# OEmiliatanO/Unpaired-Multimodal-Learning

Measured on NVIDIA B200. Metric: UML train samples/sec (img+text), higher is better.
Workload: dtype bf16

## Files before the change

### unpaired-multimodal-learning_b200/csrc/common.cuh

```cuda
#pragma once

#include <cuda.h>
#include <cuda_bf16.h>
#include <cuda_runtime.h>
#include <stdint.h>

#include <cstdio>
#include <cstring>

#include "../../include/uml_b200.h"

#if defined(__CUDA_ARCH__) && !(defined(__CUDA_ARCH_FEAT_SM100_ALL) || defined(__CUDA_ARCH_SPECIFIC__) || (__CUDA_ARCH__ >= 1000))
#error "libuml_b200 is written for sm_100a only"
#endif

namespace uml {

void set_error(const char* fmt, ...);

#define UML_FAIL(...)            \
  do {                           \
    ::uml::set_error(__VA_ARGS__); \
    return 1;                    \
  } while (0)
// ... 218 lines not shown

__device__ __forceinline__ uint32_t cluster_ctarank() {
  uint32_t r;
  asm volatile("mov.u32 %0, %%cluster_ctarank;" : "=r"(r));
  return r;
}
__device__ __forceinline__ uint32_t mapa_cta(uint32_t saddr, uint32_t rank) {
  uint32_t r;
  asm volatile("mapa.shared::cluster.u32 %0, %1, %2;" : "=r"(r) : "r"(saddr), "r"(rank));
  return r;
}
__device__ __forceinline__ void cluster_sync_all() {
  asm volatile("barrier.cluster.arrive.release.aligned;\n\tbarrier.cluster.wait.acquire.aligned;" ::: "memory");
}
__device__ __forceinline__ void mbar_arrive_remote(uint32_t cluster_addr) {
  asm volatile("mbarrier.arrive.shared::cluster.b64 _, [%0];" ::"r"(cluster_addr) : "memory");
}
__device__ __forceinline__ void tma_load_2d_cg2(void* smem_dst, const CUtensorMap* m, uint32_t bar_cluster_addr,
                                                int32_t c0, int32_t c1) {
  asm volatile(
      "cp.async.bulk.tensor.2d.cta_group::2.shared::cluster.global.mbarrier::complete_tx::bytes [%0], [%1, {%3, %4}], [%2];"
      ::"r"(smem_u32(smem_dst)), "l"(reinterpret_cast<uint64_t>(m)), "r"(bar_cluster_addr), "r"(c0), "r"(c1)
      : "memory");
}
__device__ __forceinline__ void umma_bf16_cg2(uint32_t tmem_d, uint64_t desc_a, uint64_t desc_b, uint32_t idesc,
                                              uint32_t accumulate) {
  asm volatile(
      "{\n\t.reg .pred p;\n\t"
      "setp.ne.b32 p, %4, 0;\n\t"
      "tcgen05.mma.cta_group::2.kind::f16 [%0], %1, %2, %3, p;\n\t}\n" ::"r"(tmem_d),
      "l"(desc_a), "l"(desc_b), "r"(idesc), "r"(accumulate)
      : "memory");
}
__device__ __forceinline__ void umma_commit_cg2(uint64_t* bar) {
  asm volatile(
      "tcgen05.commit.cta_group::2.mbarrier::arrive::one.shared::cluster.multicast::cluster.b64 [%0], %1;" ::"r"(
          smem_u32(bar)),
      "h"(static_cast<uint16_t>(3))
      : "memory");
}
__device__ __forceinline__ void tmem_alloc_cg2(uint32_t* smem_slot, uint32_t cols) {
  asm volatile("tcgen05.alloc.cta_group::2.sync.aligned.shared::cta.b32 [%0], %1;" ::"r"(smem_u32(smem_slot)), "r"(cols)
               : "memory");
  asm volatile("tcgen05.relinquish_alloc_permit.cta_group::2.sync.aligned;" ::: "memory");
}
__device__ __forceinline__ void tmem_dealloc_cg2(uint32_t addr, uint32_t cols) {
  asm volatile("tcgen05.dealloc.cta_group::2.sync.aligned.b32 %0, %1;" ::"r"(addr), "r"(cols) : "memory");
}

__device__ __forceinline__ float warp_sum(float v) {
#pragma unroll
  for (int o = 16; o > 0; o >>= 1) v += __shfl_xor_sync(0xffffffffu, v, o);
  return v;
}
__device__ __forceinline__ float warp_max(float v) {
#pragma unroll
  for (int o = 16; o > 0; o >>= 1) v = fmaxf(v, __shfl_xor_sync(0xffffffffu, v, o));
  return v;
}
__device__ __forceinline__ int warp_sum_i(int v) {
#pragma unroll
  for (int o = 16; o > 0; o >>= 1) v += __shfl_xor_sync(0xffffffffu, v, o);
  return v;
}

#endif

}
```

### unpaired-multimodal-learning_b200/csrc/tc_fwd2.cu

```cuda
#include <cstdlib>
#include <type_traits>

#include "common.cuh"

namespace uml {

#ifndef UML_X_TMAST
#define UML_X_TMAST 1
#endif
constexpr bool kXTmaStore = UML_X_TMAST != 0;
#ifndef UML_X_STAGES
#define UML_X_STAGES (UML_X_TMAST ? 5 : 6)
#endif
constexpr int kXStages = UML_X_STAGES;
constexpr int kXABytes = 128 * 64 * 2;
constexpr int kXBBytes = 128 * 64 * 2;
constexpr int kXStageBytes = kXABytes + kXBBytes;
constexpr int kXRecBytes = 32;
#ifndef UML_X_SLICES
#define UML_X_SLICES 2
#endif
constexpr int kXSlices = UML_X_SLICES;
constexpr int kXSliceCols = 256 / kXSlices;
#ifndef UML_X_GC
#define UML_X_GC 32
#endif
constexpr int kXGC = UML_X_GC;
#ifndef UML_X_DB
#define UML_X_DB 0
#endif
constexpr bool kXDoubleBuf = UML_X_DB != 0;
constexpr int kXGW = kXGC / 2;
constexpr int kXGroups = kXSliceCols / kXGC;
constexpr int kXHxSlots = 4;
constexpr int kXHxBytes = kXHxSlots * (kXSlices - 1) * 128 * kXRecBytes;
constexpr int kXEpiWarpsC = 4 * kXSlices;
constexpr int kXSbufWarp = 2 * 2048;
constexpr int kXSbufBytes = kXTmaStore ? kXEpiWarpsC * kXSbufWarp : 0;
constexpr int kXSmemBytes = kXStages * kXStageBytes + kXSbufBytes + kXHxBytes + 1024  + 256 ;
constexpr int kXEpiWarps = 4 * kXSlices;
constexpr int kXWarpMma = kXEpiWarps, kXWarpTma = kXEpiWarps + 1;
constexpr int kXThreads = (kXEpiWarps + 4) * 32;
#ifndef UML_X_REGS_P
#define UML_X_REGS_P (kXSlices == 2 ? 40 : 24)
#define UML_X_REGS_E (kXSlices == 2 ? 232 : 112)
#endif
constexpr int kXRegsProducer = UML_X_REGS_P, kXRegsEpilogue = UML_X_REGS_E;
static_assert((kXThreads - 128) * (kXRegsEpilogue - 168) <= 128 * (168 - kXRegsProducer) || kXSlices != 2, "setmaxnreg: the epilogue asks for more than the producers free");
#ifndef UML_X_HALF
#define UML_X_HALF (kXGroups > 2 ? kXGroups - 1 : kXGroups / 2)
#endif
constexpr int kXHalf = UML_X_HALF;
constexpr int kXMaxChunks = 4;
#ifndef UML_X_REQ_AFTER
#define UML_X_REQ_AFTER 0
#endif
constexpr int kXReqAfter = UML_X_REQ_AFTER;
static_assert(kXHalf >= 1 && kXHalf <= kXGroups && kXReqAfter < kXHalf, "the records must be requested before they are resolved");
static_assert(kXSmemBytes <= 227 * 1024, "exchange forward kernel: shared memory");

struct XSegs {
  int64_t n0;
  const float* scale_dev[2];
  float scale[2], dcoef[2];
};

struct XWork {
  float* tile_part;
  uint4* recs;
  unsigned* ctrl;
};

__device__ __forceinline__ float x_exp2(float x) {
  float y;
  asm("ex2.approx.ftz.f32 %0, %1;" : "=f"(y) : "f"(x));
  return y;
}
__device__ __forceinline__ void st_volatile_v4(uint4* p, uint32_t a, uint32_t b, uint32_t c, uint32_t d) {
  asm volatile("st.volatile.global.v4.u32 [%0], {%1, %2, %3, %4};" ::"l"(p), "r"(a), "r"(b), "r"(c), "r"(d) : "memory");
}
__device__ __forceinline__ uint4 ld_volatile_v4(const uint4* p) {
  uint4 v;
  asm volatile("ld.volatile.global.v4.u32 {%0, %1, %2, %3}, [%4];" : "=r"(v.x), "=r"(v.y), "=r"(v.z), "=r"(v.w) : "l"(p) : "memory");
  return v;
}
__device__ __forceinline__ void sts128(uint32_t a, uint32_t x, uint32_t y, uint32_t z, uint32_t w) {
  asm volatile("st.shared.v4.b32 [%0], {%1, %2, %3, %4};" ::"r"(a), "r"(x), "r"(y), "r"(z), "r"(w) : "memory");
}
__device__ __forceinline__ void sts64(uint32_t a, uint32_t x, uint32_t y) {
  asm volatile("st.shared.v2.b32 [%0], {%1, %2};" ::"r"(a), "r"(x), "r"(y) : "memory");
}
__device__ __forceinline__ uint4 lds128(uint32_t a) {
  uint4 v;
  asm volatile("ld.shared.v4.b32 {%0, %1, %2, %3}, [%4];" : "=r"(v.x), "=r"(v.y), "=r"(v.z), "=r"(v.w) : "r"(a) : "memory");
  return v;
}
__device__ __forceinline__ uint2 lds64(uint32_t a) {
  uint2 v;
  asm volatile("ld.shared.v2.b32 {%0, %1}, [%2];" : "=r"(v.x), "=r"(v.y) : "r"(a) : "memory");
  return v;
}
__device__ __forceinline__ void stg256(void* p, const uint32_t* w) {
  asm volatile("st.global.v8.b32 [%0], {%1, %2, %3, %4, %5, %6, %7, %8};" ::"l"(p), "r"(w[0]), "r"(w[1]), "r"(w[2]), "r"(w[3]),
               "r"(w[4]), "r"(w[5]), "r"(w[6]), "r"(w[7])
               : "memory");
}
__device__ __forceinline__ void named_bar_sync(int id, int n) { asm volatile("bar.sync %0, %1;" ::"r"(id), "r"(n) : "memory"); }
__device__ __forceinline__ void tmem_ld16(uint32_t taddr, uint32_t (&v)[16]) {
  asm volatile(
      "tcgen05.ld.sync.aligned.32x32b.x16.b32 "
      "{%0, %1, %2, %3, %4, %5, %6, %7, %8, %9, %10, %11, %12, %13, %14, %15}, [%16];"
      : "=r"(v[0]), "=r"(v[1]), "=r"(v[2]), "=r"(v[3]), "=r"(v[4]), "=r"(v[5]), "=r"(v[6]), "=r"(v[7]),
        "=r"(v[8]), "=r"(v[9]), "=r"(v[10]), "=r"(v[11]), "=r"(v[12]), "=r"(v[13]), "=r"(v[14]), "=r"(v[15])
      : "r"(taddr)
      : "memory");
}
__device__ __forceinline__ void tmem_ldg(uint32_t taddr, uint32_t (&v)[16]) { tmem_ld16(taddr, v); }
// ... 43 lines not shown
  case i:           \
    asm volatile("mov.b32 %0, %1;" : "=r"(r) : "r"(v[(i) < N ? (i) : 0])); \
    break;
  switch (d) {
    UML_PICK(0) UML_PICK(1) UML_PICK(2) UML_PICK(3) UML_PICK(4) UML_PICK(5) UML_PICK(6) UML_PICK(7)
    UML_PICK(8) UML_PICK(9) UML_PICK(10) UML_PICK(11) UML_PICK(12) UML_PICK(13) UML_PICK(14) UML_PICK(15)
    UML_PICK(16) UML_PICK(17) UML_PICK(18) UML_PICK(19) UML_PICK(20) UML_PICK(21) UML_PICK(22) UML_PICK(23)
    UML_PICK(24) UML_PICK(25) UML_PICK(26) UML_PICK(27) UML_PICK(28) UML_PICK(29) UML_PICK(30) UML_PICK(31)
    default: break;
  }
#undef UML_PICK
  return __uint_as_float(r);
}

template <int B, int E, class F>
__device__ __forceinline__ void static_for(F&& f) {
  if constexpr (B < E) {
    f(std::integral_constant<int, B>());
    static_for<B + 1, E>(f);
  }
}

template <bool kPred, bool kDs>
__global__ void __launch_bounds__(kXThreads, 1)
    head_fwd_ce_x_kernel(const __grid_constant__ CUtensorMap tmap_x, const __grid_constant__ CUtensorMap tmap_w,
                         const __grid_constant__ CUtensorMap tmap_g,
                         int64_t n_rows, int dim, int n_classes, int n_groups, const int32_t* __restrict__ labels, XSegs segs,
                         uint16_t* __restrict__ G, int64_t ldg, float* __restrict__ row_loss, int32_t* __restrict__ row_pred,
                         int32_t* __restrict__ row_correct, float* __restrict__ row_dscale, XWork wk) {
  extern __shared__ unsigned char smem_raw[];
  unsigned char* smem = reinterpret_cast<unsigned char*>((reinterpret_cast<uintptr_t>(smem_raw) + 1023) & ~uintptr_t(1023));
  unsigned char* sbuf = smem + kXStages * kXStageBytes;
  unsigned char* hx = sbuf + kXSbufBytes;
  uint64_t* full_bar = reinterpret_cast<uint64_t*>(hx + kXHxBytes);
  uint64_t* empty_bar = full_bar + kXStages;
  uint64_t* tfull_bar = empty_bar + kXStages;
  uint64_t* tempty_bar = tfull_bar + 2;
  uint64_t* xbar = tempty_bar + 2;
  uint32_t* tmem_slot = reinterpret_cast<uint32_t*>(xbar + 4);
  uint32_t* epoch_slot = tmem_slot + 1;
  float* run_scale = reinterpret_cast<float*>(epoch_slot + 1);

  const int warp = threadIdx.x >> 5, lane = threadIdx.x & 31;
  const uint32_t rank = cluster_ctarank();
  const bool leader = rank == 0;
  const int num_kb = (dim + 63) / 64;
  const int n_chunks = (n_classes + 255) / 256;
  const int pair = blockIdx.x >> 1;
  const int chunk = pair % n_chunks, group = pair / n_chunks;
  const int col0 = chunk * 256;
  const int n_valid = n_classes - col0 < 256 ? n_classes - col0 : 256;
  const int n_mma = ((n_valid + 15) / 16) * 16;
  const int64_t n_units = (n_rows + 255) / 256;
  const bool write_g = G != nullptr;

  if (warp == kXWarpTma && lane == 0) {
    tma_prefetch_desc(&tmap_x);
    tma_prefetch_desc(&tmap_w);
    if (kXTmaStore && write_g) tma_prefetch_desc(&tmap_g);
  }
  if (warp == kXWarpMma && lane == 0) {
    for (int s = 0; s < kXStages; ++s) {
      mbar_init(&full_bar[s], 2);
      mbar_init(&empty_bar[s], 1);
    }
    for (int b = 0; b < 2; ++b) {
      mbar_init(&tfull_bar[b], 1);
      mbar_init(&tempty_bar[b], 2 * kXEpiWarps);
    }
    for (int qq = 0; qq < 4; ++qq) mbar_init(&xbar[qq], kXSlices - 1);
    fence_barrier_init();
  }
  if (warp == kXWarpTma) tmem_alloc_cg2(tmem_slot, 512);
  tc_fence_before();
  cluster_sync_all();
  tc_fence_after();
  const uint32_t tmem_base = *tmem_slot;
  pdl_trigger();
  pdl_wait();
  if (threadIdx.x < 2) run_scale[threadIdx.x] = segs.scale_dev[threadIdx.x] ? __ldg(segs.scale_dev[threadIdx.x]) : segs.scale[threadIdx.x];
  if (threadIdx.x == 0) {
    *epoch_slot = *reinterpret_cast<volatile unsigned*>(wk.ctrl) + 1u;
    if (blockIdx.x == 0) wk.ctrl[3] = gridDim.x * 4u;
  }
  __syncthreads();
  const unsigned epoch = *epoch_slot;

  if (warp >= kXEpiWarps) {
    asm volatile("setmaxnreg.dec.sync.aligned.u32 %0;" ::"n"(kXRegsProducer));
  if (warp == kXWarpTma) {
    if (lane == 0) {
      uint32_t it = 0;
      XDBG_DECL();
      const uint32_t lead_bar0 = mapa_cta(smem_u32(&full_bar[0]), 0);
      const int32_t wrow0 = col0 + static_cast<int32_t>(rank) * (n_mma / 2);
      for (int64_t unit = group; unit < n_units; unit += n_groups) {
        const int32_t row0 = static_cast<int32_t>((unit * 2 + rank) * 128);
        for (int kb = 0; kb < num_kb; ++kb, ++it) {
          const uint32_t s = it % kXStages, ph = (it / kXStages) & 1;
          XDBG_MARK();
          mbar_wait(&empty_bar[s], ph ^ 1);
          XDBG_ACC(0);
          unsigned char* a = smem + s * kXStageBytes;
          const uint32_t lead_bar = lead_bar0 + s * 8;
#ifdef UML_X_HALFLOAD
          if (leader) mbar_arrive_expect_tx(&full_bar[s], 2 * kXBBytes);
#else
          if (leader) mbar_arrive_expect_tx(&full_bar[s], 2 * kXStageBytes);
          tma_load_2d_cg2(a, &tmap_x, lead_bar, kb * 64, row0);
#endif
          tma_load_2d_cg2(a + kXABytes, &tmap_w, lead_bar, kb * 64, wrow0);
          if (!leader) mbar_arrive_remote(lead_bar);
          XDBG_ACC(1);
        }
      }
      XDBG_FLUSH(12, 2);
    }
    __syncwarp();
  } else if (warp == kXWarpMma) {
    if (lane == 0 && leader) {
      const uint32_t idesc = make_idesc_bf16(256, static_cast<uint32_t>(n_mma), 0, 0);
      uint32_t it = 0, acc_it = 0;
      XDBG_DECL();
      for (int64_t unit = group; unit < n_units; unit += n_groups, ++acc_it) {
        const uint32_t b = acc_it & 1, aph = (acc_it >> 1) & 1;
        XDBG_MARK();
        mbar_wait(&tempty_bar[b], aph ^ 1);
        XDBG_ACC(0);
        tc_fence_after();
        const uint32_t d_tmem = tmem_base + b * 256;
        for (int kb = 0; kb < num_kb; ++kb, ++it) {
          const uint32_t s = it % kXStages, ph = (it / kXStages) & 1;
          mbar_wait(&full_bar[s], ph);
          XDBG_ACC(1);
          tc_fence_after();
          const uint32_t a_addr = smem_u32(smem + s * kXStageBytes);
          const uint32_t b_addr = a_addr + kXABytes;
#pragma unroll
          for (int k = 0; k < 4; ++k) {
            const uint64_t da = make_smem_desc(a_addr + k * 32, 16, 1024, kLayoutSw128);
            const uint64_t db = make_smem_desc(b_addr + k * 32, 16, 1024, kLayoutSw128);
            umma_bf16_cg2(d_tmem, da, db, idesc, (kb | k) != 0);
          }
          umma_commit_cg2(&empty_bar[s]);
          XDBG_ACC(2);
        }
        umma_commit_cg2(&tfull_bar[b]);
      }
      XDBG_FLUSH(9, 3);
    }
    __syncwarp();
  }
  } else {
    asm volatile("setmaxnreg.inc.sync.aligned.u32 %0;" ::"n"(kXRegsEpilogue));
    const int q = warp & 3;
    const int cq = warp >> 2;
    constexpr float kLog2e = 1.4426950408889634f;
    constexpr float kMasked = -1.0e30f;
    constexpr bool kSecond = kPred || kDs;
    const int rloc = q * 32 + lane;
    const uint32_t hx_base = smem_u32(hx);
    const uint32_t tempty_remote0 = mapa_cta(smem_u32(&tempty_bar[0]), 0);
    const int live_groups = !write_g ? 0 : static_cast<int>((ldg - col0 - cq * kXSliceCols) / kXGC);
    uint32_t tile_it = 0;
    XDBG_DECL();

    struct RowCtx {
      float sl2, sabs, sgn, dcoef, gcoef;
      bool valid, sg;
    };
    const float scale_a = run_scale[0], scale_b = run_scale[1];
    const bool any_neg = scale_a < 0.f || scale_b < 0.f;
    auto row_ctx = [&](int64_t row) {
      RowCtx c;
      c.valid = row < n_rows;
      c.sg = c.valid && row >= segs.n0;
      const float scale = c.sg ? run_scale[1] : run_scale[0];
      c.dcoef = c.sg ? segs.dcoef[1] : segs.dcoef[0];
      c.gcoef = c.dcoef * scale;
      c.sgn = scale < 0.f ? -1.f : 1.f;
      c.sabs = fabsf(scale);
      c.sl2 = c.sabs * kLog2e;
      return c;
    };

    uint32_t pk[kXSliceCols / 2];
    float p_gm[kXGroups];
#pragma unroll
    for (int g = 0; g < kXGroups; ++g) p_gm[g] = 0.f;
    float p_before = 0.f, p_lraw = 0.f, p_lab_p = 0.f, p_lab_gm = 0.f;
    int p_label = -1;
    int p_tile = -1;
    const uint4* p_rec = wk.recs;
    float f_M = 0.f, f_tc = 0.f, f_sl2 = 0.f;
    unsigned short f_patch = 0;
    bool f_store = false;
    unsigned char* f_grow = nullptr;
    float acc_loss[2] = {0.f, 0.f}, acc_ds[2] = {0.f, 0.f};
    int acc_hit[2] = {0, 0}, acc_cnt[2] = {0, 0};

    uint4 r0[kXMaxChunks], r1[kXMaxChunks];
    auto request_prev = [&]() {
      if (static_cast<int64_t>(p_tile) * 128 + rloc < n_rows) {
#pragma unroll
        for (int c2 = 0; c2 < kXMaxChunks; ++c2) {
          if (c2 < n_chunks) {
            r0[c2] = ld_volatile_v4(p_rec + c2 * 2);
            if (kSecond) r1[c2] = ld_volatile_v4(p_rec + c2 * 2 + 1);
          }
        }
      }
    };
    auto resolve_prev = [&]() {
      const int64_t row = static_cast<int64_t>(p_tile) * 128 + rloc;
      const RowCtx c = row_ctx(row);
      float M = -INFINITY, S = 0.f, PR = 0.f, before_chunks = -INFINITY;
      int garg = 0x7fffffff;
      if (c.valid) {
        for (unsigned polls = 0;; ++polls) {
          bool fresh = true;
#pragma unroll
          for (int c2 = 0; c2 < kXMaxChunks; ++c2) {
            if (c2 < n_chunks) {
              fresh = fresh && r0[c2].y == epoch && r0[c2].w == epoch;
              if (kSecond) fresh = fresh && r1[c2].y == epoch && r1[c2].w == epoch;
            }
          }
          if (fresh) break;
          if (polls > (1u << 20)) {
            atomicExch(wk.ctrl + 2, 1u);
            break;
          }
          request_prev();
        }
        float om[kXMaxChunks], os[kXMaxChunks];
#pragma unroll
        for (int c2 = 0; c2 < kXMaxChunks; ++c2) {
          om[c2] = c2 < n_chunks ? __uint_as_float(r0[c2].x) : -INFINITY;
          os[c2] = c2 < n_chunks ? __uint_as_float(r0[c2].z) : 0.f;
          M = fmaxf(M, om[c2]);
          if (c2 < chunk) before_chunks = fmaxf(before_chunks, om[c2]);
        }
        const float offM = __fmul_rn(M, c.sl2);
#pragma unroll
        for (int c2 = 0; c2 < kXMaxChunks; ++c2) {
          const float e = x_exp2(__fmul_rn(om[c2], c.sl2) - offM);
          S = fmaf(os[c2], e, S);
          if (kDs) PR = fmaf(c2 < n_chunks ? __uint_as_float(r1[c2].x) : 0.f, e, PR);
        }
        if (kPred) {
          float bestm = -INFINITY;
#pragma unroll
          for (int c2 = 0; c2 < kXMaxChunks; ++c2) {
            if (c2 < n_chunks && om[c2] > bestm) {
              bestm = om[c2];
              garg = static_cast<int>(r1[c2].z);
            }
          }
        }
      }
      f_M = __fmul_rn(M, c.sl2);
      f_sl2 = c.sl2;
      f_tc = __fdividef(c.gcoef, S);
      f_store = c.valid && live_groups > 0;
      f_grow = reinterpret_cast<unsigned char*>(G) + (row * ldg + col0 + cq * kXSliceCols) * 2;
      {
        const float f = x_exp2(__fmul_rn(p_lab_gm, c.sl2) - f_M) * f_tc;
        f_patch = __bfloat16_as_ushort(__float2bfloat16_rn(fmaf(p_lab_p, f, -c.gcoef)));
      }
      if (cq == 0) {
        const int lc_chunk = p_label - col0;
        if (c.valid && lc_chunk >= 0 && lc_chunk < 256) {
          const float loss = fmaxf(fmaf(__log2f(S), 0.6931471805599453f, -0.6931471805599453f * fmaf(p_lraw, c.sl2, -f_M)), 0.f);
          const float dsc = kDs ? (__fdividef(PR, S) - p_lraw) * c.sgn * c.dcoef : 0.f;
          const int hit = (p_lraw == M && p_lraw > fmaxf(before_chunks, p_before)) ? 1 : 0;
          if (row_loss) row_loss[row] = loss;
          if (kPred && row_pred) row_pred[row] = garg;
          if (row_correct) row_correct[row] = hit;
          if (kDs && row_dscale) row_dscale[row] = dsc;
          if (c.sg) { acc_loss[1] += loss; acc_ds[1] += dsc; acc_hit[1] += hit; acc_cnt[1] += 1; }
          else { acc_loss[0] += loss; acc_ds[0] += dsc; acc_hit[0] += hit; acc_cnt[0] += 1; }
        }
      }
    };
    auto finish_group = [&](auto gc) {
      constexpr int g = decltype(gc)::value;
      if (!f_store || g >= live_groups) return;
      const float gmx = p_gm[g];
      const float f = x_exp2(__fmul_rn(gmx, f_sl2) - f_M) * f_tc;
// ... 32 lines not shown
      }
      const uint32_t box = sbuf_w + (g & 1) * 2048, rowb = box + lane * 64, sw = (lane >> 1) & 3;
      if (lane == 0) bulk_wait_read<1>();
      __syncwarp();
#pragma unroll
      for (int j4 = 0; j4 < kXGW / 4; ++j4) sts128(rowb + ((j4 ^ sw) << 4), o[4 * j4], o[4 * j4 + 1], o[4 * j4 + 2], o[4 * j4 + 3]);
      const int lc = p_label - col0 - cq * kXSliceCols - g * kXGC;
      if (static_cast<unsigned>(lc) < static_cast<unsigned>(kXGC))
        asm volatile("st.shared.u16 [%0], %1;" ::"r"(rowb + (((lc >> 3) ^ sw) << 4) + (lc & 7) * 2), "h"(f_patch) : "memory");
      fence_proxy_async();
      __syncwarp();
#ifndef UML_X_NOSTORE
      if (lane == 0) {
        asm volatile("cp.async.bulk.tensor.2d.global.shared::cta.bulk_group [%0, {%2, %3}], [%1];" ::"l"(
                         reinterpret_cast<uint64_t>(&tmap_g)),
                     "r"(box), "r"(col0 + cq * kXSliceCols + g * kXGC), "r"(p_tile * 128 + q * 32)
                     : "memory");
        bulk_commit();
      }
#endif
    };
    auto finish_any = [&](auto gc) {
      if constexpr (kXTmaStore) finish_group_tma(gc);
      else finish_group(gc);
    };
    auto finish_rows = [&]() {
      if (kXTmaStore) return;
      const int lcol = p_label - col0 - cq * kXSliceCols;
      if (f_store && lcol >= 0 && lcol < kXSliceCols) *reinterpret_cast<volatile unsigned short*>(f_grow + lcol * 2) = f_patch;
    };

    int next_label = -1;
    {
      const int64_t frow = (static_cast<int64_t>(group) * 2 + rank) * 128 + rloc;
      if (group < n_units && frow < n_rows) next_label = __ldg(labels + frow);
    }
    for (int unit = group; unit < static_cast<int>(n_units); unit += n_groups, ++tile_it) {
      const int tile = unit * 2 + static_cast<int>(rank);
      const int64_t row = static_cast<int64_t>(tile) * 128 + rloc;
      const RowCtx c = row_ctx(row);
      const float sl2 = c.sl2, sgn = c.sgn;
      const int label = next_label;
      {
        const int64_t nrow = (static_cast<int64_t>(unit + n_groups) * 2 + rank) * 128 + rloc;
        next_label = nrow < n_rows ? __ldg(labels + nrow) : -1;
      }
#ifdef UML_X_NOLABEL
      const int lcol = -1000000;
#else
      const int lcol = label - col0 - cq * kXSliceCols;
#endif
      float run_max = -INFINITY, run_sum = 0.f, run_pr = 0.f, max_before = -INFINITY, lab_raw = -INFINITY;
      float lab_p = 0.f, lab_gm = 0.f;
      int arg = 0x7fffffff;
      float gm[kXGroups];
      const bool have_prev = p_tile >= 0;

      const uint32_t b = tile_it & 1, aph = (tile_it >> 1) & 1;
      XDBG_MARK();
      mbar_wait(&tfull_bar[b], aph);
      XDBG_ACC(0);
      tc_fence_after();
#ifdef UML_X_NOEPI
      tc_fence_before();
      __syncwarp();
      if (lane == 0) {
        if (!leader) mbar_arrive_remote(tempty_remote0 + b * 8);
        else mbar_arrive(&tempty_bar[b]);
      }
      continue;
#endif
      const uint32_t taddr = tmem_base + (static_cast<uint32_t>(q * 32) << 16) + b * 256 + cq * kXSliceCols;
      uint32_t vv[kXDoubleBuf ? 2 : 1][kXGC];
      uint32_t nk[kXGW * kXHalf];

      const uint64_t sl2x2 = pack2(sl2, sl2);
      auto run_group = [&](uint32_t (&v)[kXGC], uint32_t* out, auto gc) -> float {
// ... 69 lines not shown
          out[j] = *reinterpret_cast<const uint32_t*>(&hh);
        }
        float s0, s1;
        unpack2(fadd2(sx2, sy2), s0, s1);
        run_sum += s0 + s1;
        if (kDs) run_pr += q0 + q1;
        if (lab_here) {
          lab_p = __bfloat162float(__float2bfloat16_rn(x_exp2(__fmaf_rn(lab_raw, sl2, noff))));
          lab_gm = new_max;
        }
        return new_max;
      };

      constexpr int kB = kXDoubleBuf ? 1 : 0;
      tmem_ldg(taddr, vv[0]);
      static_for<0, kXGroups>([&](auto gc) {
        constexpr int g = decltype(gc)::value;
        constexpr bool last = g == kXGroups - 1;
        tmem_ld_wait();
        pin16(vv[g & kB]);
        if (g == 0) XDBG_ACC(1);
        if (last) {
          tc_fence_before();
          __syncwarp();
          if (lane == 0) {
            if (!leader) mbar_arrive_remote(tempty_remote0 + b * 8);
            else mbar_arrive(&tempty_bar[b]);
          }
        } else if (kXDoubleBuf) {
          tmem_ldg(taddr + kXGC * (g + 1), vv[(g + 1) & kB]);
        }
        gm[g] = run_group(vv[g & kB], g < kXHalf ? nk + kXGW * g : pk + kXGW * g, gc);
        if (!last && !kXDoubleBuf) tmem_ldg(taddr + kXGC * (g + 1), vv[0]);
        if (g == kXReqAfter && have_prev) request_prev();
        if (g == kXHalf - 1) {
          if (have_prev) {
            resolve_prev();
            static_for<0, (kXHalf + 1 < kXGroups ? kXHalf + 1 : kXGroups)>([&](auto fc) { finish_any(fc); });
          }
#pragma unroll
          for (int j = 0; j < kXGW * kXHalf; ++j) pk[j] = nk[j];
        } else if (g >= kXHalf && !last) {
          if (have_prev) finish_any(std::integral_constant<int, g + 1>());
        }
      });
      XDBG_ACC(2);
      if (have_prev) finish_rows();
      XDBG_ACC(3);

      const uint32_t hx_slot = hx_base + (tile_it & (kXHxSlots - 1)) * ((kXSlices - 1) * 128 * kXRecBytes);
      const uint4* rec_row = wk.recs + row * n_chunks * 2;
      if (cq != 0) {
        const uint32_t mine = hx_slot + ((cq - 1) * 128 + rloc) * kXRecBytes;
        sts128(mine, __float_as_uint(run_max), __float_as_uint(run_sum), __float_as_uint(max_before), __float_as_uint(lab_raw));
        if (kSecond) sts64(mine + 16, __float_as_uint(run_pr), static_cast<uint32_t>(arg));
        __syncwarp();
        if (lane == 0) mbar_arrive(&xbar[q]);
      } else {
        mbar_wait(&xbar[q], tile_it & 1);
        float cm = run_max, before_loc = max_before, lraw = lab_raw;
        constexpr int kOthers = kXSlices - 1;
        float o_max[kOthers], o_sum[kOthers], o_pr[kOthers];
        int o_arg[kOthers];
#pragma unroll
        for (int k = 0; k < kOthers; ++k) {
          const uint32_t other = hx_slot + (k * 128 + rloc) * kXRecBytes;
          const uint4 o4 = lds128(other);
          o_max[k] = __uint_as_float(o4.x);
          o_sum[k] = __uint_as_float(o4.y);
          cm = fmaxf(cm, o_max[k]);
          before_loc = fmaxf(before_loc, __uint_as_float(o4.z));
          lraw = fmaxf(lraw, __uint_as_float(o4.w));
          o_pr[k] = 0.f;
          o_arg[k] = 0;
          if (kSecond) {
            const uint2 o2 = lds64(other + 16);
            o_pr[k] = __uint_as_float(o2.x);
            o_arg[k] = static_cast<int>(o2.y);
          }
        }
        const float offc = __fmul_rn(cm, sl2);
        const float e_me = x_exp2(__fmul_rn(run_max, sl2) - offc);
        float cs = run_sum * e_me, cpr = kDs ? run_pr * e_me : 0.f;
#pragma unroll
        for (int k = 0; k < kOthers; ++k) {
          const float e = x_exp2(__fmul_rn(o_max[k], sl2) - offc);
          cs = fmaf(o_sum[k], e, cs);
          if (kDs) cpr = fmaf(o_pr[k], e, cpr);
        }
        int carg = arg;
        if (kPred) {
          float bmx = run_max;
#pragma unroll
          for (int k = 0; k < kOthers; ++k) {
            if (o_max[k] > bmx) {
              bmx = o_max[k];
              carg = o_arg[k];
            }
          }
        }
        if (c.valid) {
          uint4* rec = const_cast<uint4*>(rec_row) + chunk * 2;
          st_volatile_v4(rec, __float_as_uint(cm), epoch, __float_as_uint(cs), epoch);
          if (kSecond) st_volatile_v4(rec + 1, __float_as_uint(cpr), epoch, static_cast<uint32_t>(carg), epoch);
        }
        p_before = before_loc;
        p_lraw = lraw;
      }
      XDBG_ACC(4);
#pragma unroll
      for (int g = 0; g < kXGroups; ++g) p_gm[g] = gm[g];
      p_lab_p = lab_p; p_lab_gm = lab_gm;
      p_label = label; p_tile = tile; p_rec = rec_row;
    }
    if (p_tile >= 0) {
      XDBG_MARK();
      request_prev();
      resolve_prev();
      XDBG_ACC(5);
      static_for<0, kXGroups>([&](auto gc) { finish_any(gc); });
      finish_rows();
      XDBG_ACC(6);
    }
    if (kXTmaStore && lane == 0) bulk_wait<0>();
    if (cq == 0 && wk.tile_part) {
#pragma unroll
      for (int s2 = 0; s2 < 2; ++s2) {
        const float a = warp_sum(acc_loss[s2]), dd = kDs ? warp_sum(acc_ds[s2]) : 0.f;
        const int hh = warp_sum_i(acc_hit[s2]), cnt = warp_sum_i(acc_cnt[s2]);
        if (lane == 0)
          *reinterpret_cast<float4*>(wk.tile_part + ((static_cast<int64_t>(blockIdx.x) * 4 + q) * 2 + s2) * 4) =
              make_float4(a, dd, static_cast<float>(hh), static_cast<float>(cnt));
      }
    }
#ifdef UML_FWD_TIMING
    if (warp == 0 && lane == 0) XDBG_FLUSH(0, 9);
#endif
  }

  tc_fence_before();
  cluster_sync_all();
  if (warp == kXWarpTma) tmem_dealloc_cg2(tmem_base, 512);
  if (threadIdx.x == 0) {
    __threadfence();
    const unsigned done = atomicAdd(wk.ctrl + 1, 1u);
    if (done == gridDim.x - 1) {
      wk.ctrl[1] = 0u;
      __threadfence();
      *reinterpret_cast<volatile unsigned*>(wk.ctrl) = epoch;
    }
  }
}

__global__ void __launch_bounds__(1024)
    x_tile_stats_kernel(const float* __restrict__ tile_part, int64_t n_entries, uml_seg_stats* __restrict__ out) {
  pdl_trigger();
  pdl_wait();
  __shared__ float sh[4][32];
  const int s = blockIdx.x;
  float acc[4] = {0.f, 0.f, 0.f, 0.f};
  for (int64_t i = threadIdx.x; i < n_entries; i += blockDim.x) {
    const float* p = tile_part + (i * 2 + s) * 4;
#pragma unroll
    for (int k = 0; k < 4; ++k) acc[k] += p[k];
  }
#pragma unroll
  for (int k = 0; k < 4; ++k) {
    const float v = warp_sum(acc[k]);
    if ((threadIdx.x & 31) == 0) sh[k][threadIdx.x >> 5] = v;
  }
  __syncthreads();
  if (threadIdx.x == 0) {
    float tot[4] = {0.f, 0.f, 0.f, 0.f};
    for (int k = 0; k < 4; ++k)
      for (int w = 0; w < static_cast<int>(blockDim.x >> 5); ++w) tot[k] += sh[k][w];
    out[s].loss_mean = tot[3] > 0.f ? tot[0] / tot[3] : 0.f;
    out[s].dscale = tot[1];
    out[s].correct = static_cast<int32_t>(tot[2] + 0.5f);
    out[s].n = static_cast<int32_t>(tot[3] + 0.5f);
  }
}

__global__ void __launch_bounds__(1024)
    x_tile_stats_dev_kernel(const float* __restrict__ tile_part, const unsigned* __restrict__ ctrl, uml_seg_stats* __restrict__ out) {
  pdl_trigger();
  pdl_wait();
  __shared__ float sh[4][32];
  const int s = blockIdx.x;
  const int64_t n_entries = ctrl[3];
  float acc[4] = {0.f, 0.f, 0.f, 0.f};
  for (int64_t i = threadIdx.x; i < n_entries; i += blockDim.x) {
    const float* p = tile_part + (i * 2 + s) * 4;
#pragma unroll
    for (int k = 0; k < 4; ++k) acc[k] += p[k];
  }
#pragma unroll
  for (int k = 0; k < 4; ++k) {
    const float v = warp_sum(acc[k]);
    if ((threadIdx.x & 31) == 0) sh[k][threadIdx.x >> 5] = v;
  }
  __syncthreads();
  if (threadIdx.x == 0) {
    float tot[4] = {0.f, 0.f, 0.f, 0.f};
    for (int k = 0; k < 4; ++k)
      for (int w = 0; w < static_cast<int>(blockDim.x >> 5); ++w) tot[k] += sh[k][w];
    out[s].loss_mean = tot[3] > 0.f ? tot[0] / tot[3] : 0.f;
    out[s].dscale = tot[1];
    out[s].correct = static_cast<int32_t>(tot[2] + 0.5f);
    out[s].n = static_cast<int32_t>(tot[3] + 0.5f);
  }
}

struct XLayout {
  unsigned* ctrl;
  float* tile_part;
  uint4* recs;
  int64_t part_entries;
  int64_t n_groups;
};
static XLayout x_layout(float* tile_ws, int64_t n_rows, int n_classes) {
  const int64_t units = (n_rows + 255) / 256;
  const int n_chunks = (n_classes + 255) / 256;
  XLayout l;
  l.ctrl = reinterpret_cast<unsigned*>(tile_ws);
  l.tile_part = tile_ws + 16 + units * 8;
  l.recs = reinterpret_cast<uint4*>(l.tile_part + units * 256);
  l.n_groups = (sm_count() / 2) / n_chunks;
  if (l.n_groups > units) l.n_groups = units;
  l.part_entries = l.n_groups * n_chunks * 2 * 4;
  return l;
}

}

bool uml_fwd_x_eligible(int64_t n_rows, int32_t n_classes) {
  static int mode = -1;
  if (mode < 0) {
    const char* e = getenv("UML_FWD_IMPL");
    mode = (e && e[0] == 'o') ? 0 : 1;
  }
  return mode == 1 && n_rows > 128 && n_classes <= uml::kXMaxChunks * 256;
}

void uml_fwd_x_partials(float* tile_ws, int64_t n_rows, int32_t n_classes, const float** part, int64_t* n_entries) {
  const uml::XLayout l = uml::x_layout(tile_ws, n_rows, n_classes);
  *part = l.tile_part;
  *n_entries = l.part_entries;
}

int uml_head_fwd_ce_x_bf16(const uint16_t* X, int64_t n_rows, int32_t dim, const uint16_t* W, int32_t n_classes,
                           const int32_t* labels, const uml_tc_segments* segs, uint16_t* G, int64_t ldg, float* row_loss,
                           int32_t* row_pred, int32_t* row_correct, float* row_dscale, float* tile_ws, uml_seg_stats* stats,
                           void* stream) {
  using namespace uml;
  UML_REQUIRE(X && W && labels && segs && tile_ws && n_rows > 0 && dim > 0 && n_classes > 0, "head_fwd_ce_x: bad arguments");
  UML_REQUIRE(dim % 8 == 0, "head_fwd_ce_x: dim (%d) must be a multiple of 8 (16-byte bf16 rows for TMA)", dim);
  UML_REQUIRE(n_classes <= kXMaxChunks * 256, "head_fwd_ce_x: at most %d classes", kXMaxChunks * 256);
  UML_REQUIRE(!G || (ldg % 64 == 0 && ldg >= n_classes && ldg <= kXMaxChunks * 256),
              "head_fwd_ce_x: ldg must be a multiple of 64 and >= n_classes");
  UML_REQUIRE(segs->nseg >= 1 && segs->nseg <= UML_MAX_SEGMENTS, "head_fwd_ce_x: 1..2 segments");
// ... 7 lines not shown
  if (make_tmap_2d(&tw, W, CU_TENSOR_MAP_DATA_TYPE_BFLOAT16, 2, dim, n_classes, static_cast<uint64_t>(dim) * 2, 64, 128,
                   CU_TENSOR_MAP_SWIZZLE_128B))
    return 1;
  CUtensorMap tg = tx;
  if (kXTmaStore && G &&
      make_tmap_2d(&tg, G, CU_TENSOR_MAP_DATA_TYPE_BFLOAT16, 2, static_cast<uint64_t>(ldg), n_rows, static_cast<uint64_t>(ldg) * 2, 32, 32,
                   CU_TENSOR_MAP_SWIZZLE_64B))
    return 1;
  XSegs fs;
  fs.n0 = segs->nseg > 1 ? n0 : INT64_MAX;
  bool learnable = false;
  for (int i = 0; i < 2; ++i) {
    const int j = i < segs->nseg ? i : 0;
    const double n = static_cast<double>(segs->seg_rows[j] > 0 ? segs->seg_rows[j] : 1);
    fs.scale[i] = segs->scale[j];
    fs.scale_dev[i] = segs->scale_dev[j];
    fs.dcoef[i] = static_cast<float>(static_cast<double>(segs->loss_weight[j]) / n);
    learnable = learnable || segs->scale_dev[j] != nullptr;
  }
  const bool ds = learnable || row_dscale != nullptr;
  using Kern = void (*)(CUtensorMap, CUtensorMap, CUtensorMap, int64_t, int, int, int, const int32_t*, XSegs, uint16_t*, int64_t, float*,
                        int32_t*, int32_t*, float*, XWork);
  const int slot = (row_pred ? 2 : 0) + (ds ? 1 : 0);
  const Kern kerns[4] = {head_fwd_ce_x_kernel<false, false>, head_fwd_ce_x_kernel<false, true>,
                         head_fwd_ce_x_kernel<true, false>, head_fwd_ce_x_kernel<true, true>};
  static bool attr_set[4] = {false, false, false, false};
  if (!attr_set[slot]) {
    UML_CUDA(cudaFuncSetAttribute(kerns[slot], cudaFuncAttributeMaxDynamicSharedMemorySize, kXSmemBytes));
    attr_set[slot] = true;
  }
  const int n_chunks = (n_classes + 255) / 256;
  const XLayout l = x_layout(tile_ws, n_rows, n_classes);
  const int64_t n_groups = l.n_groups;
  UML_REQUIRE(n_groups >= 1, "head_fwd_ce_x: the device has too few SMs for %d class chunks", n_chunks);
  XWork wk;
  wk.tile_part = l.tile_part;
  wk.recs = l.recs;
  wk.ctrl = l.ctrl;
  const dim3 grid(static_cast<unsigned>(n_groups * n_chunks * 2));
  UML_CUDA(launch_kernel(kerns[slot], grid, dim3(kXThreads), kXSmemBytes, as_stream(stream), 2, kPdlFwd, tx, tw, tg, n_rows,
                         static_cast<int>(dim), static_cast<int>(n_classes), static_cast<int>(n_groups), labels, fs, G, ldg,
                         row_loss, row_pred, row_correct, row_dscale, wk));
  if (stats)
    UML_CUDA(launch_kernel(x_tile_stats_kernel, dim3(segs->nseg), dim3(1024), 0, as_stream(stream), 1, kPdlStats,
                           static_cast<const float*>(l.tile_part), l.part_entries, stats));
  return 0;
}

int uml_fwd_x_reduce_stats(float* tile_ws, int64_t n_rows, int32_t nseg, uml_seg_stats* stats, void* stream) {
  using namespace uml;
  const XLayout l = x_layout(tile_ws, n_rows, 1);
  UML_CUDA(launch_kernel(x_tile_stats_dev_kernel, dim3(nseg), dim3(1024), 0, as_stream(stream), 1, kPdlStats,
                         static_cast<const float*>(l.tile_part), static_cast<const unsigned*>(l.ctrl), stats));
  return 0;
}

extern "C" {

#ifdef UML_FWD_TIMING
int uml_debug_fwdx_timing(long long* host_out , int reset) {
  if (reset) {
    static long long zeros[148 * 16];
    return cudaMemcpyToSymbol(uml::g_fwdx_dbg, zeros, sizeof(zeros)) != cudaSuccess;
  }
  return cudaMemcpyFromSymbol(host_out, uml::g_fwdx_dbg, sizeof(long long) * 148 * 16) != cudaSuccess;
}
#endif

int uml_fwd_x_failed(const float* tile_ws) {
  unsigned v = 0;
  if (cudaMemcpy(&v, reinterpret_cast<const unsigned*>(tile_ws) + 2, sizeof(v), cudaMemcpyDeviceToHost) != cudaSuccess) return -1;
  return v != 0 ? 1 : 0;
}
// ... 3 lines not shown
```

Before: 311.9 million.

## Exchange per-chunk softmax records via cluster DSMEM and multicast X tiles

The cluster grows from a CTA pair to 2×n_chunks CTAs, so every class-chunk pair for a row tile sits in one cluster. Per-row max/sum records now travel to peers through st.async into a double-buffered shared-memory ring guarded by mbarriers, replacing epoch-tagged volatile global stores and polling. The X activation tile is loaded once per k-block and multicast to all chunk pairs, with the stage-release barrier counting all of them. This cuts global-memory traffic and spin latency in the cross-chunk reduction, but the larger clusters can fit fewer groups and tie every pair's pipeline together.

```diff
diff --git a/unpaired-multimodal-learning_b200/csrc/common.cuh b/unpaired-multimodal-learning_b200/csrc/common.cuh
--- a/unpaired-multimodal-learning_b200/csrc/common.cuh
+++ b/unpaired-multimodal-learning_b200/csrc/common.cuh
@@ -274,11 +274,25 @@
       "l"(desc_a), "l"(desc_b), "r"(idesc), "r"(accumulate)
       : "memory");
 }
-__device__ __forceinline__ void umma_commit_cg2(uint64_t* bar) {
+__device__ __forceinline__ void tma_load_2d_cg2_mc(void* smem_dst, const CUtensorMap* m, uint32_t bar_leader_addr, int32_t c0,
+                                                   int32_t c1, uint16_t cta_mask) {
+  asm volatile(
+      "cp.async.bulk.tensor.2d.cta_group::2.shared::cluster.global.mbarrier::complete_tx::bytes.multicast::cluster"
+      " [%0], [%1, {%3, %4}], [%2], %5;"
+      ::"r"(smem_u32(smem_dst)), "l"(reinterpret_cast<uint64_t>(m)), "r"(bar_leader_addr), "r"(c0), "r"(c1), "h"(cta_mask)
+      : "memory");
+}
+__device__ __forceinline__ void st_async_v4(uint32_t cluster_addr, uint32_t cluster_bar, uint32_t a, uint32_t b, uint32_t c,
+                                            uint32_t d) {
+  asm volatile("st.async.shared::cluster.mbarrier::complete_tx::bytes.v4.b32 [%0], {%2, %3, %4, %5}, [%1];" ::"r"(cluster_addr),
+               "r"(cluster_bar), "r"(a), "r"(b), "r"(c), "r"(d)
+               : "memory");
+}
+__device__ __forceinline__ void umma_commit_cg2(uint64_t* bar, uint16_t cta_mask = 3) {
   asm volatile(
       "tcgen05.commit.cta_group::2.mbarrier::arrive::one.shared::cluster.multicast::cluster.b64 [%0], %1;" ::"r"(
           smem_u32(bar)),
-      "h"(static_cast<uint16_t>(3))
+      "h"(cta_mask)
       : "memory");
 }
 __device__ __forceinline__ void tmem_alloc_cg2(uint32_t* smem_slot, uint32_t cols) {
diff --git a/unpaired-multimodal-learning_b200/csrc/tc_fwd2.cu b/unpaired-multimodal-learning_b200/csrc/tc_fwd2.cu
--- a/unpaired-multimodal-learning_b200/csrc/tc_fwd2.cu
+++ b/unpaired-multimodal-learning_b200/csrc/tc_fwd2.cu
@@ -37,7 +37,10 @@
 constexpr int kXEpiWarpsC = 4 * kXSlices;
 constexpr int kXSbufWarp = 2 * 2048;
 constexpr int kXSbufBytes = kXTmaStore ? kXEpiWarpsC * kXSbufWarp : 0;
-constexpr int kXSmemBytes = kXStages * kXStageBytes + kXSbufBytes + kXHxBytes + 1024  + 256 ;
+constexpr int kXMaxChunks = 4;
+constexpr int kXRingSlotBytes = kXMaxChunks * 128 * 16;
+constexpr int kXRingBytes = 2 * kXRingSlotBytes;
+constexpr int kXSmemBytes = kXStages * kXStageBytes + kXSbufBytes + kXHxBytes + kXRingBytes + 1024  + 256 ;
 constexpr int kXEpiWarps = 4 * kXSlices;
 constexpr int kXWarpMma = kXEpiWarps, kXWarpTma = kXEpiWarps + 1;
 constexpr int kXThreads = (kXEpiWarps + 4) * 32;
@@ -51,12 +54,7 @@
 #define UML_X_HALF (kXGroups > 2 ? kXGroups - 1 : kXGroups / 2)
 #endif
 constexpr int kXHalf = UML_X_HALF;
-constexpr int kXMaxChunks = 4;
-#ifndef UML_X_REQ_AFTER
-#define UML_X_REQ_AFTER 0
-#endif
-constexpr int kXReqAfter = UML_X_REQ_AFTER;
-static_assert(kXHalf >= 1 && kXHalf <= kXGroups && kXReqAfter < kXHalf, "the records must be requested before they are resolved");
+static_assert(kXHalf >= 1 && kXHalf <= kXGroups, "the previous unit is finished during the new one");
 static_assert(kXSmemBytes <= 227 * 1024, "exchange forward kernel: shared memory");
 
 struct XSegs {
@@ -67,7 +65,6 @@
 
 struct XWork {
   float* tile_part;
-  uint4* recs;
   unsigned* ctrl;
 };
 
@@ -76,13 +73,21 @@
   asm("ex2.approx.ftz.f32 %0, %1;" : "=f"(y) : "f"(x));
   return y;
 }
-__device__ __forceinline__ void st_volatile_v4(uint4* p, uint32_t a, uint32_t b, uint32_t c, uint32_t d) {
-  asm volatile("st.volatile.global.v4.u32 [%0], {%1, %2, %3, %4};" ::"l"(p), "r"(a), "r"(b), "r"(c), "r"(d) : "memory");
-}
-__device__ __forceinline__ uint4 ld_volatile_v4(const uint4* p) {
-  uint4 v;
-  asm volatile("ld.volatile.global.v4.u32 {%0, %1, %2, %3}, [%4];" : "=r"(v.x), "=r"(v.y), "=r"(v.z), "=r"(v.w) : "l"(p) : "memory");
-  return v;
+__device__ __forceinline__ bool mbar_wait_bounded(uint32_t bar, uint32_t parity) {
+  long long t0 = 0;
+  for (;;) {
+    uint32_t ok;
+    asm volatile(
+        "{\n\t.reg .pred p;\n\t"
+        "mbarrier.try_wait.parity.shared::cta.b64 p, [%1], %2;\n\t"
+        "selp.u32 %0, 1, 0, p;\n\t}\n"
+        : "=r"(ok)
+        : "r"(bar), "r"(parity)
+        : "memory");
+    if (ok) return true;
+    if (t0 == 0) t0 = clock64();
+    else if (clock64() - t0 > 2000000000ll) return false;
+  }
 }
 __device__ __forceinline__ void sts128(uint32_t a, uint32_t x, uint32_t y, uint32_t z, uint32_t w) {
   asm volatile("st.shared.v4.b32 [%0], {%1, %2, %3, %4};" ::"r"(a), "r"(x), "r"(y), "r"(z), "r"(w) : "memory");
@@ -192,22 +197,23 @@
   unsigned char* smem = reinterpret_cast<unsigned char*>((reinterpret_cast<uintptr_t>(smem_raw) + 1023) & ~uintptr_t(1023));
   unsigned char* sbuf = smem + kXStages * kXStageBytes;
   unsigned char* hx = sbuf + kXSbufBytes;
-  uint64_t* full_bar = reinterpret_cast<uint64_t*>(hx + kXHxBytes);
+  unsigned char* ring = hx + kXHxBytes;
+  uint64_t* full_bar = reinterpret_cast<uint64_t*>(ring + kXRingBytes);
   uint64_t* empty_bar = full_bar + kXStages;
   uint64_t* tfull_bar = empty_bar + kXStages;
   uint64_t* tempty_bar = tfull_bar + 2;
   uint64_t* xbar = tempty_bar + 2;
-  uint32_t* tmem_slot = reinterpret_cast<uint32_t*>(xbar + 4);
-  uint32_t* epoch_slot = tmem_slot + 1;
-  float* run_scale = reinterpret_cast<float*>(epoch_slot + 1);
+  uint64_t* rbar = xbar + 4;
+  uint32_t* tmem_slot = reinterpret_cast<uint32_t*>(rbar + 8);
+  float* run_scale = reinterpret_cast<float*>(tmem_slot + 1);
 
   const int warp = threadIdx.x >> 5, lane = threadIdx.x & 31;
   const uint32_t rank = cluster_ctarank();
-  const bool leader = rank == 0;
+  const uint32_t half = rank & 1, lead_rank = rank & ~1u;
+  const bool leader = half == 0;
   const int num_kb = (dim + 63) / 64;
   const int n_chunks = (n_classes + 255) / 256;
-  const int pair = blockIdx.x >> 1;
-  const int chunk = pair % n_chunks, group = pair / n_chunks;
+  const int chunk = static_cast<int>(rank >> 1), group = static_cast<int>(blockIdx.x) / (2 * n_chunks);
   const int col0 = chunk * 256;
   const int n_valid = n_classes - col0 < 256 ? n_classes - col0 : 256;
   const int n_mma = ((n_valid + 15) / 16) * 16;
@@ -222,13 +228,14 @@
   if (warp == kXWarpMma && lane == 0) {
     for (int s = 0; s < kXStages; ++s) {
       mbar_init(&full_bar[s], 2);
-      mbar_init(&empty_bar[s], 1);
+      mbar_init(&empty_bar[s], n_chunks);
     }
     for (int b = 0; b < 2; ++b) {
       mbar_init(&tfull_bar[b], 1);
       mbar_init(&tempty_bar[b], 2 * kXEpiWarps);
     }
     for (int qq = 0; qq < 4; ++qq) mbar_init(&xbar[qq], kXSlices - 1);
+    for (int i = 0; i < 8; ++i) mbar_init(&rbar[i], 1);
     fence_barrier_init();
   }
   if (warp == kXWarpTma) tmem_alloc_cg2(tmem_slot, 512);
@@ -239,12 +246,8 @@
   pdl_trigger();
   pdl_wait();
   if (threadIdx.x < 2) run_scale[threadIdx.x] = segs.scale_dev[threadIdx.x] ? __ldg(segs.scale_dev[threadIdx.x]) : segs.scale[threadIdx.x];
-  if (threadIdx.x == 0) {
-    *epoch_slot = *reinterpret_cast<volatile unsigned*>(wk.ctrl) + 1u;
-    if (blockIdx.x == 0) wk.ctrl[3] = gridDim.x * 4u;
-  }
+  if (threadIdx.x == 0 && blockIdx.x == 0) wk.ctrl[3] = gridDim.x * 4u;
   __syncthreads();
-  const unsigned epoch = *epoch_slot;
 
   if (warp >= kXEpiWarps) {
     asm volatile("setmaxnreg.dec.sync.aligned.u32 %0;" ::"n"(kXRegsProducer));
@@ -252,10 +255,11 @@
     if (lane == 0) {
       uint32_t it = 0;
       XDBG_DECL();
-      const uint32_t lead_bar0 = mapa_cta(smem_u32(&full_bar[0]), 0);
-      const int32_t wrow0 = col0 + static_cast<int32_t>(rank) * (n_mma / 2);
+      const uint32_t lead_bar0 = mapa_cta(smem_u32(&full_bar[0]), lead_rank);
+      const int32_t wrow0 = col0 + static_cast<int32_t>(half) * (n_mma / 2);
+      const uint16_t xmask = static_cast<uint16_t>((0x5555u << half) & ((1u << (2 * n_chunks)) - 1u));
       for (int64_t unit = group; unit < n_units; unit += n_groups) {
-        const int32_t row0 = static_cast<int32_t>((unit * 2 + rank) * 128);
+        const int32_t row0 = static_cast<int32_t>((unit * 2 + half) * 128);
         for (int kb = 0; kb < num_kb; ++kb, ++it) {
           const uint32_t s = it % kXStages, ph = (it / kXStages) & 1;
           XDBG_MARK();
@@ -267,7 +271,8 @@
           if (leader) mbar_arrive_expect_tx(&full_bar[s], 2 * kXBBytes);
 #else
           if (leader) mbar_arrive_expect_tx(&full_bar[s], 2 * kXStageBytes);
-          tma_load_2d_cg2(a, &tmap_x, lead_bar, kb * 64, row0);
+          if (n_chunks == 1) tma_load_2d_cg2(a, &tmap_x, lead_bar, kb * 64, row0);
+          else if (kb % n_chunks == chunk) tma_load_2d_cg2_mc(a, &tmap_x, smem_u32(&full_bar[s]) & 0xFEFFFFFFu, kb * 64, row0, xmask);
 #endif
           tma_load_2d_cg2(a + kXABytes, &tmap_w, lead_bar, kb * 64, wrow0);
           if (!leader) mbar_arrive_remote(lead_bar);
@@ -280,6 +285,7 @@
   } else if (warp == kXWarpMma) {
     if (lane == 0 && leader) {
       const uint32_t idesc = make_idesc_bf16(256, static_cast<uint32_t>(n_mma), 0, 0);
+      const uint16_t all_mask = static_cast<uint16_t>((1u << (2 * n_chunks)) - 1u), pair_mask = static_cast<uint16_t>(3u << lead_rank);
       uint32_t it = 0, acc_it = 0;
       XDBG_DECL();
       for (int64_t unit = group; unit < n_units; unit += n_groups, ++acc_it) {
@@ -302,10 +308,10 @@
             const uint64_t db = make_smem_desc(b_addr + k * 32, 16, 1024, kLayoutSw128);
             umma_bf16_cg2(d_tmem, da, db, idesc, (kb | k) != 0);
           }
-          umma_commit_cg2(&empty_bar[s]);
+          umma_commit_cg2(&empty_bar[s], all_mask);
           XDBG_ACC(2);
         }
-        umma_commit_cg2(&tfull_bar[b]);
+        umma_commit_cg2(&tfull_bar[b], pair_mask);
       }
       XDBG_FLUSH(9, 3);
     }
@@ -320,7 +326,13 @@
     constexpr bool kSecond = kPred || kDs;
     const int rloc = q * 32 + lane;
     const uint32_t hx_base = smem_u32(hx);
-    const uint32_t tempty_remote0 = mapa_cta(smem_u32(&tempty_bar[0]), 0);
+    const uint32_t tempty_remote0 = mapa_cta(smem_u32(&tempty_bar[0]), lead_rank);
+    const uint32_t ring_base = smem_u32(ring), rbar_q = smem_u32(&rbar[q]);
+    constexpr uint32_t kRingTx = 32 * 16;
+    if (cq == 0 && lane == 0) {
+      mbar_arrive_expect_tx(&rbar[q], n_chunks * kRingTx);
+      mbar_arrive_expect_tx(&rbar[4 + q], n_chunks * kRingTx);
+    }
     const int live_groups = !write_g ? 0 : static_cast<int>((ldg - col0 - cq * kXSliceCols) / kXGC);
     uint32_t tile_it = 0;
     XDBG_DECL();
@@ -351,7 +363,7 @@
     float p_before = 0.f, p_lraw = 0.f, p_lab_p = 0.f, p_lab_gm = 0.f;
     int p_label = -1;
     int p_tile = -1;
-    const uint4* p_rec = wk.recs;
+    uint32_t p_it = 0;
     float f_M = 0.f, f_tc = 0.f, f_sl2 = 0.f;
     unsigned short f_patch = 0;
     bool f_store = false;
@@ -359,45 +371,25 @@
     float acc_loss[2] = {0.f, 0.f}, acc_ds[2] = {0.f, 0.f};
     int acc_hit[2] = {0, 0}, acc_cnt[2] = {0, 0};
 
-    uint4 r0[kXMaxChunks], r1[kXMaxChunks];
-    auto request_prev = [&]() {
-      if (static_cast<int64_t>(p_tile) * 128 + rloc < n_rows) {
-#pragma unroll
-        for (int c2 = 0; c2 < kXMaxChunks; ++c2) {
-          if (c2 < n_chunks) {
-            r0[c2] = ld_volatile_v4(p_rec + c2 * 2);
-            if (kSecond) r1[c2] = ld_volatile_v4(p_rec + c2 * 2 + 1);
-          }
-        }
-      }
-    };
     auto resolve_prev = [&]() {
       const int64_t row = static_cast<int64_t>(p_tile) * 128 + rloc;
       const RowCtx c = row_ctx(row);
       float M = -INFINITY, S = 0.f, PR = 0.f, before_chunks = -INFINITY;
       int garg = 0x7fffffff;
+      const uint32_t slot = p_it & 1;
+      if (!mbar_wait_bounded(rbar_q + slot * 32, (p_it >> 1) & 1)) atomicExch(wk.ctrl + 2, 1u);
+      if (cq == 0) {
+        __syncwarp();
+        if (lane == 0) mbar_arrive_expect_tx(&rbar[slot * 4 + q], n_chunks * kRingTx);
+      }
       if (c.valid) {
-        for (unsigned polls = 0;; ++polls) {
-          bool fresh = true;
-#pragma unroll
-          for (int c2 = 0; c2 < kXMaxChunks; ++c2) {
-            if (c2 < n_chunks) {
-              fresh = fresh && r0[c2].y == epoch && r0[c2].w == epoch;
-              if (kSecond) fresh = fresh && r1[c2].y == epoch && r1[c2].w == epoch;
-            }
-          }
-          if (fresh) break;
-          if (polls > (1u << 20)) {
-            atomicExch(wk.ctrl + 2, 1u);
-            break;
-          }
-          request_prev();
-        }
+        uint4 r[kXMaxChunks];
         float om[kXMaxChunks], os[kXMaxChunks];
 #pragma unroll
         for (int c2 = 0; c2 < kXMaxChunks; ++c2) {
-          om[c2] = c2 < n_chunks ? __uint_as_float(r0[c2].x) : -INFINITY;
-          os[c2] = c2 < n_chunks ? __uint_as_float(r0[c2].z) : 0.f;
+          if (c2 < n_chunks) r[c2] = lds128(ring_base + slot * kXRingSlotBytes + (c2 * 128 + rloc) * 16);
+          om[c2] = c2 < n_chunks ? __uint_as_float(r[c2].x) : -INFINITY;
+          os[c2] = c2 < n_chunks ? __uint_as_float(r[c2].y) : 0.f;
           M = fmaxf(M, om[c2]);
           if (c2 < chunk) before_chunks = fmaxf(before_chunks, om[c2]);
         }
@@ -406,7 +398,7 @@
         for (int c2 = 0; c2 < kXMaxChunks; ++c2) {
           const float e = x_exp2(__fmul_rn(om[c2], c.sl2) - offM);
           S = fmaf(os[c2], e, S);
-          if (kDs) PR = fmaf(c2 < n_chunks ? __uint_as_float(r1[c2].x) : 0.f, e, PR);
+          if (kDs) PR = fmaf(c2 < n_chunks ? __uint_as_float(r[c2].z) : 0.f, e, PR);
         }
         if (kPred) {
           float bestm = -INFINITY;
@@ -414,7 +406,7 @@
           for (int c2 = 0; c2 < kXMaxChunks; ++c2) {
             if (c2 < n_chunks && om[c2] > bestm) {
               bestm = om[c2];
-              garg = static_cast<int>(r1[c2].z);
+              garg = static_cast<int>(r[c2].w);
             }
           }
         }
@@ -513,17 +505,17 @@
 
     int next_label = -1;
     {
-      const int64_t frow = (static_cast<int64_t>(group) * 2 + rank) * 128 + rloc;
+      const int64_t frow = (static_cast<int64_t>(group) * 2 + half) * 128 + rloc;
       if (group < n_units && frow < n_rows) next_label = __ldg(labels + frow);
     }
     for (int unit = group; unit < static_cast<int>(n_units); unit += n_groups, ++tile_it) {
-      const int tile = unit * 2 + static_cast<int>(rank);
+      const int tile = unit * 2 + static_cast<int>(half);
       const int64_t row = static_cast<int64_t>(tile) * 128 + rloc;
       const RowCtx c = row_ctx(row);
       const float sl2 = c.sl2, sgn = c.sgn;
       const int label = next_label;
       {
-        const int64_t nrow = (static_cast<int64_t>(unit + n_groups) * 2 + rank) * 128 + rloc;
+        const int64_t nrow = (static_cast<int64_t>(unit + n_groups) * 2 + half) * 128 + rloc;
         next_label = nrow < n_rows ? __ldg(labels + nrow) : -1;
       }
 #ifdef UML_X_NOLABEL
@@ -659,7 +651,6 @@
         }
         gm[g] = run_group(vv[g & kB], g < kXHalf ? nk + kXGW * g : pk + kXGW * g, gc);
         if (!last && !kXDoubleBuf) tmem_ldg(taddr + kXGC * (g + 1), vv[0]);
-        if (g == kXReqAfter && have_prev) request_prev();
         if (g == kXHalf - 1) {
           if (have_prev) {
             resolve_prev();
@@ -676,7 +667,6 @@
       XDBG_ACC(3);
 
       const uint32_t hx_slot = hx_base + (tile_it & (kXHxSlots - 1)) * ((kXSlices - 1) * 128 * kXRecBytes);
-      const uint4* rec_row = wk.recs + row * n_chunks * 2;
       if (cq != 0) {
         const uint32_t mine = hx_slot + ((cq - 1) * 128 + rloc) * kXRecBytes;
         sts128(mine, __float_as_uint(run_max), __float_as_uint(run_sum), __float_as_uint(max_before), __float_as_uint(lab_raw));
@@ -726,10 +716,17 @@
             }
           }
         }
-        if (c.valid) {
-          uint4* rec = const_cast<uint4*>(rec_row) + chunk * 2;
-          st_volatile_v4(rec, __float_as_uint(cm), epoch, __float_as_uint(cs), epoch);
-          if (kSecond) st_volatile_v4(rec + 1, __float_as_uint(cpr), epoch, static_cast<uint32_t>(carg), epoch);
+        {
+          const uint32_t slot = tile_it & 1;
+          const uint32_t dst = ring_base + slot * kXRingSlotBytes + (chunk * 128 + rloc) * 16, bar = rbar_q + slot * 32;
+#pragma unroll
+          for (int c2 = 0; c2 < kXMaxChunks; ++c2) {
+            if (c2 < n_chunks) {
+              const uint32_t to = 2 * c2 + half;
+              st_async_v4(mapa_cta(dst, to), mapa_cta(bar, to), __float_as_uint(cm), __float_as_uint(cs), __float_as_uint(cpr),
+                          static_cast<uint32_t>(carg));
+            }
+          }
         }
         p_before = before_loc;
         p_lraw = lraw;
@@ -738,11 +735,10 @@
 #pragma unroll
       for (int g = 0; g < kXGroups; ++g) p_gm[g] = gm[g];
       p_lab_p = lab_p; p_lab_gm = lab_gm;
-      p_label = label; p_tile = tile; p_rec = rec_row;
+      p_label = label; p_tile = tile; p_it = tile_it;
     }
     if (p_tile >= 0) {
       XDBG_MARK();
-      request_prev();
       resolve_prev();
       XDBG_ACC(5);
       static_for<0, kXGroups>([&](auto gc) { finish_any(gc); });
@@ -768,15 +764,6 @@
   tc_fence_before();
   cluster_sync_all();
   if (warp == kXWarpTma) tmem_dealloc_cg2(tmem_base, 512);
-  if (threadIdx.x == 0) {
-    __threadfence();
-    const unsigned done = atomicAdd(wk.ctrl + 1, 1u);
-    if (done == gridDim.x - 1) {
-      wk.ctrl[1] = 0u;
-      __threadfence();
-      *reinterpret_cast<volatile unsigned*>(wk.ctrl) = epoch;
-    }
-  }
 }
 
 __global__ void __launch_bounds__(1024)
@@ -838,10 +825,34 @@
   }
 }
 
+static int x_max_clusters(int n_chunks) {
+  static int cached[64][kXMaxChunks + 1] = {};
+  int dev = 0;
+  if (cudaGetDevice(&dev) != cudaSuccess || dev < 0 || dev >= 64) return 0;
+  int& n = cached[dev][n_chunks];
+  if (n == 0) {
+    auto kern = head_fwd_ce_x_kernel<false, false>;
+    if (cudaFuncSetAttribute(kern, cudaFuncAttributeMaxDynamicSharedMemorySize, kXSmemBytes) != cudaSuccess) return 0;
+    cudaLaunchConfig_t cfg;
+    memset(&cfg, 0, sizeof(cfg));
+    cfg.gridDim = dim3(2 * n_chunks);
+    cfg.blockDim = dim3(kXThreads);
+    cfg.dynamicSmemBytes = kXSmemBytes;
+    cudaLaunchAttribute attr;
+    attr.id = cudaLaunchAttributeClusterDimension;
+    attr.val.clusterDim.x = 2 * n_chunks;
+    attr.val.clusterDim.y = 1;
+    attr.val.clusterDim.z = 1;
+    cfg.attrs = &attr;
+    cfg.numAttrs = 1;
+    if (cudaOccupancyMaxActiveClusters(&n, kern, &cfg) != cudaSuccess) n = 0;
+  }
+  return n;
+}
+
 struct XLayout {
   unsigned* ctrl;
   float* tile_part;
-  uint4* recs;
   int64_t part_entries;
   int64_t n_groups;
 };
@@ -851,8 +862,7 @@
   XLayout l;
   l.ctrl = reinterpret_cast<unsigned*>(tile_ws);
   l.tile_part = tile_ws + 16 + units * 8;
-  l.recs = reinterpret_cast<uint4*>(l.tile_part + units * 256);
-  l.n_groups = (sm_count() / 2) / n_chunks;
+  l.n_groups = x_max_clusters(n_chunks);
   if (l.n_groups > units) l.n_groups = units;
   l.part_entries = l.n_groups * n_chunks * 2 * 4;
   return l;
@@ -926,13 +936,12 @@
   const int n_chunks = (n_classes + 255) / 256;
   const XLayout l = x_layout(tile_ws, n_rows, n_classes);
   const int64_t n_groups = l.n_groups;
-  UML_REQUIRE(n_groups >= 1, "head_fwd_ce_x: the device has too few SMs for %d class chunks", n_chunks);
+  UML_REQUIRE(n_groups >= 1, "head_fwd_ce_x: the device holds no cluster of %d CTAs for %d class chunks", 2 * n_chunks, n_chunks);
   XWork wk;
   wk.tile_part = l.tile_part;
-  wk.recs = l.recs;
   wk.ctrl = l.ctrl;
   const dim3 grid(static_cast<unsigned>(n_groups * n_chunks * 2));
-  UML_CUDA(launch_kernel(kerns[slot], grid, dim3(kXThreads), kXSmemBytes, as_stream(stream), 2, kPdlFwd, tx, tw, tg, n_rows,
+  UML_CUDA(launch_kernel(kerns[slot], grid, dim3(kXThreads), kXSmemBytes, as_stream(stream), 2 * n_chunks, kPdlFwd, tx, tw, tg, n_rows,
                          static_cast<int>(dim), static_cast<int>(n_classes), static_cast<int>(n_groups), labels, fs, G, ldg,
                          row_loss, row_pred, row_correct, row_dscale, wk));
   if (stats)
```

Result: faster. 317.7 million, median of 6 (+1.9%).
